# AIRLegend/ChessRL

Measured on AMD Instinct MI355X. Metric: MCTS simulations/sec at 800 sims/move, higher is better.
Workload: dtype f16

## Files before the change

### chessrl_amd/csrc/tower_x16.hpp

```cpp
#pragma once
#include "tower_common.hpp"

namespace crl_tower {

template <int F, int NB_, int SPLIT_ = 0>
struct Geo16 {
    static_assert(F == 64 || F == 128 || F == 256, "supported filter counts");
    static constexpr int SPLIT = SPLIT_;
    static constexpr int LO_OFF = F * 2;
    static constexpr int NB = NB_;
    static constexpr int WPB = 8 / NB;
    static constexpr int NT = (F == 64 && NB == 2) ? 1 : 2;
    static constexpr int CT = 2 * NT;
    static constexpr int CG = F / (16 * CT);
    static constexpr int PH = WPB / CG;
    static constexpr int PT = 4 / PH;
    static_assert(NB * CG * PH == 8 && (PH == 1 || PH == 2), "8 waves per workgroup");
    static constexpr int KT = F == 256 ? 32 : 64;
    static constexpr int SPT = KT / 32;
    static constexpr int WROW = KT * 2;
    static constexpr int WCH = WROW / 16;
    static constexpr int TILE_BYTES = F * WROW;
    static constexpr int GL = TILE_BYTES / 8192;
    static constexpr int AROW_CH = (SPLIT ? 2 * F : F) < 128 ? 128 : (SPLIT ? 2 * F : F);
    static constexpr int AROW = AROW_CH * 2 + 32;
    static constexpr int ABOARD = 64 * AROW;
    static constexpr int ZERO_OFF = NB * ABOARD;
    static constexpr int ZSTRIDE = AROW;
    static constexpr int ZERO_BYTES = 16 * ZSTRIDE;
    static constexpr int BIAS_OFF = ZERO_OFF + ZERO_BYTES;
    static constexpr int WRING_OFF = ((BIAS_OFF + 2 * F * 4 + 1023) / 1024) * 1024;
    static constexpr int LDS_BYTES = WRING_OFF + PIPE_RING * TILE_BYTES;
    static_assert(LDS_BYTES <= 160 * 1024, "LDS budget");
    static constexpr int lds_bytes(int ring) { return WRING_OFF + ring * TILE_BYTES; }
    static constexpr int WPLANE = F * 64;
    __device__ static int wswz(int row) { return (0 - (row >> 2)) & 3; }
    __host__ __device__ static constexpr int chan_of(int ct, int i)
    {
        return 32 * (ct >> 1) + 8 * (i >> 2) + 4 * (ct & 1) + (i & 3);
    }
    __host__ __device__ static constexpr int row_channel(int row)
    {
        return (row & ~31) + chan_of((row >> 4) & 1, row & 15);
    }
};

constexpr int GROUP_TAPS = 3;
template <int NB, int PAIR, int GROUP>
constexpr int ring_slots()
{
    return GROUP ? GROUP_TAPS * (NB == 2 ? 4 : 3) : (PAIR ? 5 : PIPE_RING);
}

template <class G>
__device__ inline void stage_wtile_x16(const unsigned char *wts, lds_byte *lds, int t, int tid, int wave_u,
                                       int slot = -1)
{
    const unsigned char *src = wts + (size_t)t * G::TILE_BYTES;
    const int slot0 = G::WRING_OFF + (slot < 0 ? (t & (PIPE_RING - 1)) : slot) * G::TILE_BYTES;
    const int dst0 = slot0 + wave_u * 1024;
#pragma unroll
    for (int j = 0; j < G::GL; j++) {
        const int idx = j * 512 + tid;
        const unsigned off = (unsigned)(idx * 16);
        __builtin_amdgcn_global_load_lds(
            (const __attribute__((address_space(1))) void *)(src + off),
            (__attribute__((address_space(3))) void *)(lds + dst0 + j * 8192), 16, 0, 0);
    }
}

template <class G, int F>
__device__ inline void stage_bias_x16(const float *bias, lds_byte *lds, int conv, int lane, int wave_u)
{
    if (wave_u >= F / 64) return;
    const unsigned long long a = reinterpret_cast<unsigned long long>(bias + (size_t)conv * F + wave_u * 64);
    const unsigned lo = __builtin_amdgcn_readfirstlane((unsigned)a), hi = __builtin_amdgcn_readfirstlane((unsigned)(a >> 32));
    const unsigned char *src = reinterpret_cast<const unsigned char *>(((unsigned long long)hi << 32) | lo);
    __builtin_amdgcn_global_load_lds(
        (const __attribute__((address_space(1))) void *)(src + (unsigned)(lane * 4)),
        (__attribute__((address_space(3))) void *)(lds + G::BIAS_OFF + (conv & 1) * F * 4 + wave_u * 256), 4, 0, 0);
}

typedef float f32x4v __attribute__((ext_vector_type(4)));

#ifndef CRL_TRUNK_RANKPAIR
#define CRL_TRUNK_RANKPAIR 1
#endif
template <int F, int NB, int PAIR, int GROUP, int SPLIT, int IDX>
struct RankTiles {
    static constexpr bool value = CRL_TRUNK_RANKPAIR != 0 && F == 128 && NB == 4 && PAIR == 1 && GROUP == 0 &&
                                  SPLIT == 0 && IDX == 0;
};

template <int F, int NB, int BITS = 0, int ALT = 0, int PAIR = 0, int GROUP = 0, int SPLIT = 0, int IDX = 0>
__global__ __launch_bounds__(512, 2) void k_trunk_x16(const unsigned char *__restrict__ planes,
                                                       const unsigned char *__restrict__ wts,
                                                       const float *__restrict__ bias,
                                                       float *__restrict__ out, int n_blocks,
                                                       const float *__restrict__ head_w,
                                                       const float *__restrict__ head_b,
                                                       float *__restrict__ head_out)
{
    static_assert(ALT == 0, "reserved");
    typedef Geo16<F, NB, SPLIT> G;
    static_assert(!SPLIT || !GROUP, "split precision runs the plain / pair pipelines");
    constexpr int PT = G::PT, CT = G::CT;
    extern __shared__ __attribute__((aligned(1024))) unsigned char lds_raw[];
    lds_byte *lds = (lds_byte *)lds_raw;
    const int lds_base = (int)(size_t)lds;
    const int tid = threadIdx.x, lane = tid & 63, wave = tid >> 6;
    const int board_w = wave / G::WPB;
    const int obase = (16 * CT) * ((wave / G::PH) % G::CG);
    const int pbase = 32 * (wave % G::PH);
    const int r = lane & 15, q = lane >> 4;
    const int wave_u = __builtin_amdgcn_readfirstlane(wave);
    constexpr bool RP = RankTiles<F, NB, PAIR, GROUP, SPLIT, IDX>::value;
    const int rp_half = wave_u >> 2;
    const int board = RP ? 2 * ((wave >> 1) & 1) + (r >> 3) : board_w;
    const int pos0 = RP ? (rp_half ? 56 : 0) + (r & 7) : pbase + r;
    const int pstep = RP ? (rp_half ? -8 : 8) : 16;
    const int n_convs = 1 + 2 * n_blocks;
    const int tiles_stem = 9 * (SPLIT ? 2 : 1) * (128 / G::KT), tiles_conv = 9 * (SPLIT ? 2 : 1) * (F / G::KT);
    const int n_tiles = tiles_stem + 2 * n_blocks * tiles_conv;
    const size_t wg_board0 = (size_t)blockIdx.x * G::NB;
    int rows[G::NB];
    if constexpr (IDX) {
        static_assert(BITS == 1, "the indexed launch reads plane bitboards");
        const int *list = reinterpret_cast<const int *>(out);
        const int listed = __builtin_amdgcn_readfirstlane(list[0]);
        if ((int)wg_board0 >= listed) return;
#pragma unroll
        for (int b = 0; b < G::NB; b++) {
            const int k = (int)wg_board0 + b < listed ? (int)wg_board0 + b : listed - 1;
            rows[b] = __builtin_amdgcn_readfirstlane(list[LIST_HEADER + k]);
        }
    }

    static_assert(!PAIR || F == 128 || F == 256, "pair publishing: even tile counts per layer");
    constexpr int GK = GROUP_TAPS;
    constexpr int GR = ring_slots<NB, PAIR, GROUP>();
    constexpr int GRG = GR / GK;
    static_assert(G::lds_bytes(GR) <= 160 * 1024, "LDS budget");
    static_assert(!GROUP || (F == 64 && !PAIR && G::SPT == 2 && G::GL == 1 && 2 * (PT + CT) < 16),
                  "group pipeline: 64 filters");
    stage_bias_x16<G, F>(bias, lds, 0, lane, wave_u);
    if constexpr (GROUP) {
#pragma unroll
        for (int k = 0; k < GK * (GRG - 1); k++) stage_wtile_x16<G>(wts, lds, k, tid, wave_u, k);
    } else {
        stage_wtile_x16<G>(wts, lds, 0, tid, wave_u, PAIR ? 0 : -1);
        stage_wtile_x16<G>(wts, lds, 1, tid, wave_u, PAIR ? 1 : -1);
        stage_wtile_x16<G>(wts, lds, 2, tid, wave_u, PAIR ? 2 : -1);
        if constexpr (PAIR) stage_wtile_x16<G>(wts, lds, 3, tid, wave_u, 3);
    }

    {
        if constexpr (IDX) {
            expand_bitplanes_rows<G::NB, G::AROW, G::ABOARD>(planes, lds, rows, tid);
        } else if constexpr (BITS) {
            expand_bitplanes<G::NB, G::AROW, G::ABOARD>(planes, lds, wg_board0, tid);
        } else {
            const u32x4 *src = reinterpret_cast<const u32x4 *>(planes + wg_board0 * BOARD_BYTES);
#pragma unroll
            for (int i = 0; i < G::NB * 2; i++) {
                const int c16 = i * 512 + tid;
                const int p = (c16 >> 4) & 63, c = c16 & 15, b = c16 >> 10;
                u32x4 v = src[c16];
                *reinterpret_cast<__attribute__((address_space(3))) u32x4 *>(
                    lds + b * G::ABOARD + p * G::AROW + (c << 4)) = v;
            }
        }
        for (int i = tid; i < G::ZERO_BYTES / 16; i += 512)
            *reinterpret_cast<__attribute__((address_space(3))) u32x4 *>(lds + G::ZERO_OFF + i * 16) =
                u32x4{0u, 0u, 0u, 0u};
    }
    if constexpr (GROUP) wait_vmcnt<GK * (GRG - 2)>();
    else wait_vmcnt<2 * G::GL>();
    wait_lgkm<0>();
    __builtin_amdgcn_s_barrier();
    __builtin_amdgcn_sched_barrier(0);

    const int px = r & 7, py0 = (pbase >> 3) + (r >> 3);
    const int base0 = lds_base + board * G::ABOARD + pos0 * G::AROW + q * 16;
    const int zero_q = lds_base + G::ZERO_OFF + q * 16;
    const int act_row0 = board * G::ABOARD + pos0 * G::AROW;
    const int row_step = pstep * G::AROW;
    const unsigned long long xm_left = __ballot(px >= 1), xm_right = __ballot(px <= 6);
    unsigned long long ym_up[PT], ym_down[PT];
#pragma unroll
    for (int pt = 0; pt < PT; pt++) {
        ym_up[pt] = RP ? ~0ull : __ballot(py0 + 2 * pt >= 1);
        ym_down[pt] = RP ? ~0ull : __ballot(py0 + 2 * pt <= 6);
    }
    const int w0 = lds_base + G::WRING_OFF + (obase + r) * 64 + ((q ^ G::wswz(obase + r)) << 4);
    static_assert((16 * 64) == 1024 && G::TILE_BYTES * 2 + G::WPLANE + 3 * 1024 < 65536, "ds_read immediate");

    f32x4v res[PT][CT];
#pragma unroll
    for (int a = 0; a < PT; a++)
#pragma unroll
        for (int b = 0; b < CT; b++) res[a][b] = f32x4v{-0.f, -0.f, -0.f, -0.f};

    constexpr int HP = PT / 2;

    int t = 0;
    int slot_tap = 0;
    auto slot_add = [](int s, int k) { const int x = s + k; return x >= 5 ? x - 5 : x; };
    for (int conv = 0; conv < n_convs; conv++) {
        f32x4v acc[PT][CT];
#pragma unroll
        for (int ct = 0; ct < CT; ct++) {
            const f32x4 bv = *reinterpret_cast<const __attribute__((address_space(3))) f32x4 *>(
                lds + G::BIAS_OFF + (conv & 1) * F * 4 + (obase + G::chan_of(ct, 0) + 8 * q) * 4);
#pragma unroll
            for (int pt = 0; pt < PT; pt++) acc[pt][ct] = f32x4v{bv[0], bv[1], bv[2], bv[3]};
        }
        bool bias_staged = false;

        half8 xa[HP], xb[HP], w[2][CT];
        int ab[2][PT];

        auto run_tap = [&](auto NSC, auto DUPC, bool first_tap, bool last_tap, auto SKC, auto NSKC) {
            constexpr int NS = decltype(NSC)::value, DUP = decltype(DUPC)::value;
            constexpr int SK = decltype(SKC)::value ? 1 : 0, NSK = decltype(NSKC)::value ? 1 : 0;
            static_assert(RP || (SK == 0 && NSK == 0), "whole blocks leave the board only with rank tiles");
            static_assert(DUP == 1 || (SPLIT && DUP == 2), "shared weight sub-steps belong to the split kernels");
            const int t_tap0 = t;
            auto fetch_xa = [&](auto IC, bool next_tap, auto SC) {
                constexpr int i = decltype(IC)::value;
#pragma unroll
                for (int pt = decltype(SC)::value; pt < HP; pt++)
                    xa[pt] = lds_read16_asm<(i / DUP) * 64 + (i % DUP) * G::LO_OFF>(ab[next_tap ? 1 : 0][pt]);
            };
            auto fetch_xb = [&](auto IC) {
                constexpr int i = decltype(IC)::value;
#pragma unroll
                for (int pt = 0; pt < HP; pt++)
                    xb[pt] = lds_read16_asm<(i / DUP) * 64 + (i % DUP) * G::LO_OFF>(ab[0][HP + pt]);
            };
            constexpr int NSW = NS / DUP;
            constexpr int TPT = NSW / G::SPT;
            static_assert((TPT == 1 || TPT == 2 || TPT == 4) && PIPE_RING == 4 && NSW % 2 == 0, "ring");
            int wv[PAIR ? TPT : 1], wv_nxt;
            if constexpr (PAIR) {
#pragma unroll
                for (int k = 0; k < TPT; k++) wv[k] = w0 + slot_add(slot_tap, k) * G::TILE_BYTES;
                wv_nxt = w0 + slot_add(slot_tap, TPT) * G::TILE_BYTES;
            } else {
                wv[0] = w0 + (t_tap0 & (PIPE_RING - 1)) * G::TILE_BYTES;
                wv_nxt = w0 + ((t_tap0 + TPT) & (PIPE_RING - 1)) * G::TILE_BYTES;
            }
            auto fetch_w1 = [&](auto IC, auto CC, bool next_tap, half8 (&dst)[CT]) {
                constexpr int i = decltype(IC)::value, ct = decltype(CC)::value;
                constexpr int off = ct * 1024 + (i % G::SPT) * G::WPLANE + (PAIR ? 0 : (i / G::SPT) * G::TILE_BYTES);
                dst[ct] = lds_read16_asm<off>(next_tap ? wv_nxt : wv[PAIR ? i / G::SPT : 0]);
            };
            auto fetch_w = [&](auto IC, bool next_tap, half8 (&dst)[CT]) {
                static_for<0, CT>([&](auto CC) { fetch_w1(IC, CC, next_tap, dst); });
            };
            if (first_tap) {
                fetch_xa(std::integral_constant<int, 0>{}, false, std::integral_constant<int, SK>{});
                fetch_w(std::integral_constant<int, 0>{}, false, w[0]);
            }
            static_for<0, NS>([&](auto IC) {
                constexpr int i = decltype(IC)::value;
                constexpr int wi = i / DUP;
                constexpr bool w_first = i % DUP == 0, w_last = i % DUP == DUP - 1;
                constexpr int s = wi % G::SPT;
                constexpr int cur = wi % 2, nxt = 1 - cur;
                if constexpr (!w_first) {
                } else if constexpr (PAIR) {
                    if constexpr (s == G::SPT - 1 && ((wi / G::SPT) & 1) == 1) {
                        wait_vmcnt<0>();
                        __builtin_amdgcn_s_barrier();
                        __builtin_amdgcn_sched_barrier(0);
                        if (!bias_staged) {
                            bias_staged = true;
                            if (conv + 1 < n_convs) stage_bias_x16<G, F>(bias, lds, conv + 1, lane, wave_u);
                        }
                        const int slot_cur = slot_add(slot_tap, wi / G::SPT);
                        if (t + 3 < n_tiles) stage_wtile_x16<G>(wts, lds, t + 3, tid, wave_u, slot_add(slot_cur, 3));
                        if (t + 4 < n_tiles) stage_wtile_x16<G>(wts, lds, t + 4, tid, wave_u, slot_add(slot_cur, 4));
                    }
                } else if constexpr (s == G::SPT - 1) {
                    if (t + 2 < n_tiles) wait_vmcnt<G::GL>();
                    else wait_vmcnt<0>();
                    __builtin_amdgcn_s_barrier();
                    __builtin_amdgcn_sched_barrier(0);
                    if (!bias_staged) {
                        bias_staged = true;
                        if (conv + 1 < n_convs) stage_bias_x16<G, F>(bias, lds, conv + 1, lane, wave_u);
                    }
                    if (t + 3 < n_tiles) stage_wtile_x16<G>(wts, lds, t + 3, tid, wave_u);
                }
                fetch_xb(IC);
                wait_lgkm<HP>();
                __builtin_amdgcn_sched_barrier(0);
#pragma unroll
                for (int pt = SK; pt < HP; pt++)
#pragma unroll
                    for (int ct = 0; ct < CT; ct++)
                        acc[pt][ct] = __builtin_amdgcn_mfma_f32_16x16x32_f16(w[cur][ct], xa[pt], acc[pt][ct], 0, 0, 0);
                __builtin_amdgcn_sched_barrier(0);
                constexpr bool wrap = i + 1 >= NS;
                bool issued = false;
                if (!wrap || !last_tap) {
                    issued = true;
                    if constexpr (wrap) fetch_xa(std::integral_constant<int, 0>{}, true, std::integral_constant<int, NSK>{});
                    else fetch_xa(std::integral_constant<int, i + 1>{}, false, std::integral_constant<int, SK>{});
                }
                if (!issued) wait_lgkm<0>();
                else wait_lgkm<HP - (wrap ? NSK : SK)>();
                __builtin_amdgcn_sched_barrier(0);
                static_for<0, HP * CT>([&](auto KC) {
                    constexpr int k = decltype(KC)::value, pt = k / CT, ct = k % CT;
                    acc[HP + pt][ct] = __builtin_amdgcn_mfma_f32_16x16x32_f16(w[cur][ct], xb[pt], acc[HP + pt][ct], 0, 0, 0);
                    if constexpr (k < CT && w_last) {
                        __builtin_amdgcn_sched_barrier(0);
                        if (issued) {
                            if constexpr (wrap) fetch_w1(std::integral_constant<int, 0>{}, KC, true, w[nxt]);
                            else fetch_w1(std::integral_constant<int, wi + 1>{}, KC, false, w[nxt]);
                        }
                        __builtin_amdgcn_sched_barrier(0);
                    }
                });
                __builtin_amdgcn_sched_barrier(0);
                if constexpr (s == G::SPT - 1 && w_last) t++;
            });
        };

        const int hshift = GROUP ? (conv == 0 ? 1 : 0) : ((conv != 0 && F == 256) ? 1 : 0);
        constexpr int chstep = GROUP ? 128 : 256;
        const int parts = SPLIT ? 2 : 1;
        const int per_tap = parts << hshift;
        const int nv = 9 * per_tap;
        int base0_tap = base0, r_tap = r;
        auto vtap_rows = [&](int v, int (&dst)[PT]) {
            int tap, choff;
            if constexpr (SPLIT) {
                tap = v / per_tap;
                const int rem = v - tap * per_tap;
                choff = (rem & ((1 << hshift) - 1)) * chstep;
            } else {
                tap = v >> hshift;
                choff = (v & ((1 << hshift) - 1)) * chstep;
            }
            const int dy = tap / 3 - 1, dx = tap % 3 - 1;
            const int shift = 8 * dy + dx;
            const int zrow = zero_q + ((r_tap + shift) & 15) * G::ZSTRIDE + choff;
            const int inb = base0_tap + shift * G::AROW + choff;
            const unsigned long long xm = dx < 0 ? xm_left : (dx > 0 ? xm_right : ~0ull);
#pragma unroll
            for (int pt = 0; pt < PT; pt++) {
                const unsigned long long m = xm & (dy < 0 ? ym_up[pt] : (dy > 0 ? ym_down[pt] : ~0ull));
                const int row = inb + pt * row_step;
                asm("v_cndmask_b32 %0, %1, %2, %3" : "=v"(dst[pt]) : "v"(zrow), "v"(row), "s"(m));
            }
        };
        if constexpr (GROUP) {
            constexpr int FR = PT + CT;
            half8 fx[3][PT], fw[3][CT];
            const int n_groups = n_tiles / GK;
            for (int g0 = 0; g0 < nv; g0 += GK) {
                const bool more = g0 + GK < nv;
                int rows[GK + 1][PT], wb[GK + 1];
#pragma unroll
                for (int k = 0; k <= GK; k++) {
                    vtap_rows(g0 + k < nv ? g0 + k : 0, rows[k]);
                    int slot = slot_tap + k;
                    slot = slot >= GR ? slot - GR : slot;
                    wb[k] = w0 + slot * G::TILE_BYTES;
                }
                auto fetch = [&](auto JC) {
                    constexpr int j = decltype(JC)::value, b = j % 3, k = j / 2, pl = j % 2;
#pragma unroll
                    for (int pt = 0; pt < PT; pt++) fx[b][pt] = lds_read16_asm<pl * 64>(rows[k][pt]);
                    static_for<0, CT>([&](auto CC) {
                        constexpr int ct = decltype(CC)::value;
                        fw[b][ct] = lds_read16_asm<ct * 1024 + pl * G::WPLANE>(wb[k]);
                    });
                };
                if (g0 == 0) {
                    fetch(std::integral_constant<int, 0>{});
                    fetch(std::integral_constant<int, 1>{});
                }
                static_for<0, 2 * GK>([&](auto IC) {
                    constexpr int i = decltype(IC)::value;
                    if constexpr (i == 2 * GK - 2) {
                        const int tg = t / GK;
                        if (tg + 1 < n_groups) {
                            if (tg + GRG - 2 < n_groups) wait_vmcnt<GK * (GRG - 3)>();
                            else wait_vmcnt<0>();
                            __builtin_amdgcn_s_barrier();
                            __builtin_amdgcn_sched_barrier(0);
                            if (!bias_staged) {
                                bias_staged = true;
                                if (conv + 1 < n_convs) stage_bias_x16<G, F>(bias, lds, conv + 1, lane, wave_u);
                            }
                            if (tg + GRG - 1 < n_groups) {
                                int slot = slot_tap - GK;
                                slot = slot < 0 ? slot + GR : slot;
#pragma unroll
                                for (int k = 0; k < GK; k++)
                                    stage_wtile_x16<G>(wts, lds, (tg + GRG - 1) * GK + k, tid, wave_u, slot + k);
                            }
                        }
                    }
                    if constexpr (i + 2 < 2 * GK) fetch(std::integral_constant<int, i + 2>{});
                    else if (more) fetch(std::integral_constant<int, i + 2>{});
                    if constexpr (i + 2 < 2 * GK) wait_lgkm<2 * FR>();
                    else if constexpr (i == 2 * GK - 2) { if (more) wait_lgkm<2 * FR>(); else wait_lgkm<FR>(); }
                    else { if (more) wait_lgkm<2 * FR>(); else wait_lgkm<0>(); }
                    __builtin_amdgcn_sched_barrier(0);
#pragma unroll
                    for (int pt = 0; pt < PT; pt++)
#pragma unroll
                        for (int ct = 0; ct < CT; ct++)
                            acc[pt][ct] = __builtin_amdgcn_mfma_f32_16x16x32_f16(fw[i % 3][ct], fx[i % 3][pt], acc[pt][ct], 0, 0, 0);
                    __builtin_amdgcn_sched_barrier(0);
                });
                t += GK;
                slot_tap += GK;
                slot_tap = slot_tap >= GR ? slot_tap - GR : slot_tap;
            }
        } else if constexpr (RP) {
            constexpr std::integral_constant<int, 1> once{};
            auto run_conv = [&](auto HC) {
                constexpr int hh = decltype(HC)::value;
                auto fresh = [&] {
                    base0_tap = base0;
                    r_tap = r;
                    asm volatile("" : "+v"(base0_tap), "+v"(r_tap));
                };
                fresh();
                vtap_rows(0, ab[1]);
                static_for<0, 9>([&](auto VC) {
                    constexpr int v = decltype(VC)::value;
                    constexpr bool sk = hh == 0 ? v < 3 : v >= 6;
                    constexpr bool nsk = v + 1 < 9 && (hh == 0 ? v + 1 < 3 : v + 1 >= 6);
#pragma unroll
                    for (int pt = 0; pt < PT; pt++) ab[0][pt] = ab[1][pt];
                    fresh();
                    vtap_rows(v + 1 < 9 ? v + 1 : 0, ab[1]);
                    run_tap(std::integral_constant<int, 4>{}, once, v == 0, v == 8, std::integral_constant<bool, sk>{},
                            std::integral_constant<bool, nsk>{});
                    slot_tap = slot_add(slot_tap, 4 / G::SPT);
                });
            };
            if (rp_half == 0) run_conv(std::integral_constant<int, 0>{});
            else run_conv(std::integral_constant<int, 1>{});
        } else {
        constexpr std::false_type nsk{};
        vtap_rows(0, ab[1]);
        for (int v = 0; v < nv; v++) {
#pragma unroll
            for (int pt = 0; pt < PT; pt++) ab[0][pt] = ab[1][pt];
            vtap_rows(v + 1 < nv ? v + 1 : 0, ab[1]);
            constexpr std::integral_constant<int, 1> once{};
            bool whi_twice = false;
            if constexpr (SPLIT) {
                const bool whi = ((v % per_tap) >> hshift) == 0;
                whi_twice = conv != 0 && whi;
            }
            if (whi_twice) {
                if constexpr (SPLIT) {
                    constexpr std::integral_constant<int, 2> twice{};
                    if (F == 64) run_tap(std::integral_constant<int, 4>{}, twice, v == 0, v == nv - 1, nsk, nsk);
                    else run_tap(std::integral_constant<int, 8>{}, twice, v == 0, v == nv - 1, nsk, nsk);
                }
            } else if (F == 64 && conv != 0) run_tap(std::integral_constant<int, 2>{}, once, v == 0, v == nv - 1, nsk, nsk);
            else run_tap(std::integral_constant<int, 4>{}, once, v == 0, v == nv - 1, nsk, nsk);
            if constexpr (PAIR) slot_tap = slot_add(slot_tap, 4 / G::SPT);
            if constexpr (SPLIT) wait_lgkm<0>();
        }
        }

        wait_lgkm<0>();
        __builtin_amdgcn_s_barrier();
        __builtin_amdgcn_sched_barrier(0);
        const bool conv1 = (conv & 1) != 0;
        const float floor = conv == 0 ? -__builtin_inff() : 0.f;
        auto store_pair = [&](int pt, int g, const half4 &lo, const half4 &hi) {
            *reinterpret_cast<__attribute__((address_space(3))) half8 *>(
                lds + act_row0 + pt * row_step + (obase + 32 * g + 8 * q) * 2) =
                half8{lo[0], lo[1], lo[2], lo[3], hi[0], hi[1], hi[2], hi[3]};
        };
        const half4 zero4 = {(_Float16)0, (_Float16)0, (_Float16)0, (_Float16)0};
        auto store_split = [&](int pt, int g, const f32x4v &a, const f32x4v &b) {
            half8 hi8, lo8;
#pragma unroll
            for (int j = 0; j < 4; j++) {
                hi8[j] = (_Float16)a[j];
                hi8[4 + j] = (_Float16)b[j];
                lo8[j] = (_Float16)(a[j] - (float)hi8[j]);
                lo8[4 + j] = (_Float16)(b[j] - (float)hi8[4 + j]);
            }
            lds_byte *dst = lds + act_row0 + pt * row_step + (obase + 32 * g + 8 * q) * 2;
            *reinterpret_cast<__attribute__((address_space(3))) half8 *>(dst) = hi8;
            *reinterpret_cast<__attribute__((address_space(3))) half8 *>(dst + G::LO_OFF) = lo8;
        };
        if constexpr (SPLIT) {
            auto write_layer = [&](auto value) {
#pragma unroll
                for (int g = 0; g < CT / 2; g++)
#pragma unroll
                    for (int pt = 0; pt < PT; pt++) store_split(pt, g, value(pt, 2 * g), value(pt, 2 * g + 1));
            };
            if (conv1) {
                write_layer([&](int pt, int ct) {
                    f32x4v o;
#pragma unroll
                    for (int j = 0; j < 4; j++) o[j] = fmaxf(acc[pt][ct][j], 0.f);
                    return o;
                });
                asm volatile("; conv1 written");
            } else {
                write_layer([&](int pt, int ct) {
                    const f32x4v sum = acc[pt][ct] + res[pt][ct];
#pragma unroll
                    for (int j = 0; j < 4; j++) res[pt][ct][j] = fmaxf(sum[j], floor);
                    return res[pt][ct];
                });
                asm volatile("; conv2 written");
            }
        } else
        if (conv1) {
#pragma unroll
            for (int g = 0; g < CT / 2; g++)
#pragma unroll
                for (int pt = 0; pt < PT; pt++) {
                    half4 o16[2];
#pragma unroll
                    for (int h = 0; h < 2; h++) {
#pragma unroll
                        for (int j = 0; j < 4; j++) o16[h][j] = (_Float16)acc[pt][2 * g + h][j];
                        o16[h] = __builtin_elementwise_max(o16[h], zero4);
                    }
                    store_pair(pt, g, o16[0], o16[1]);
                }
        } else {
#pragma unroll
            for (int g = 0; g < CT / 2; g++)
#pragma unroll
                for (int pt = 0; pt < PT; pt++) {
                    half4 o16[2];
#pragma unroll
                    for (int h = 0; h < 2; h++) {
                        const int ct = 2 * g + h;
                        const f32x4v sum = acc[pt][ct] + res[pt][ct];
#pragma unroll
                        for (int j = 0; j < 4; j++) {
                            const float v = fmaxf(sum[j], floor);
                            res[pt][ct][j] = v;
                            o16[h][j] = (_Float16)v;
                        }
                    }
                    store_pair(pt, g, o16[0], o16[1]);
                }
        }
        wait_lgkm<0>();
        __builtin_amdgcn_s_barrier();
        __builtin_amdgcn_sched_barrier(0);
    }
    if (!IDX && out) {
#pragma unroll
        for (int pt = 0; pt < PT; pt++) {
            const int p = pos0 + pstep * pt;
#pragma unroll
            for (int ct = 0; ct < CT; ct++) {
                const int o0 = obase + G::chan_of(ct, 0) + 8 * q;
                f32x4 v;
#pragma unroll
                for (int j = 0; j < 4; j++) v[j] = res[pt][ct][j];
                *reinterpret_cast<f32x4 *>(out + ((wg_board0 + board) * 64 + p) * F + o0) = v;
            }
        }
    }

    if (head_out) {
        constexpr int NC = 4 * G::CG;
        float part[PT][3];
#pragma unroll
        for (int pt = 0; pt < PT; pt++)
#pragma unroll
            for (int k = 0; k < 3; k++) part[pt][k] = 0.f;
#pragma unroll
        for (int ct = 0; ct < CT; ct++) {
            const int o0 = obase + G::chan_of(ct, 0) + 8 * q;
#pragma unroll
            for (int k = 0; k < 3; k++) {
                const f32x4 wv = *reinterpret_cast<const f32x4 *>(head_w + k * F + o0);
#pragma unroll
                for (int pt = 0; pt < PT; pt++)
#pragma unroll
                    for (int j = 0; j < 4; j++) part[pt][k] += res[pt][ct][j] * wv[j];
            }
        }
        __attribute__((address_space(3))) float *scratch = (__attribute__((address_space(3))) float *)lds;
#pragma unroll
        for (int pt = 0; pt < PT; pt++)
#pragma unroll
            for (int k = 0; k < 3; k++)
                scratch[(((board * 64 + pos0 + pstep * pt) * 3) + k) * NC + (obase / (16 * CT)) * 4 + q] = part[pt][k];
        wait_lgkm<0>();
        __builtin_amdgcn_s_barrier();
        for (int i = tid; i < G::NB * 64 * 3; i += 512) {
            const int k = i % 3, bp = i / 3;
            float v = 0.f;
#pragma unroll
            for (int c = 0; c < NC; c++) v += scratch[i * NC + c];
            v += head_b[k];
            size_t gb = wg_board0 + (bp >> 6);
            if constexpr (IDX) {
                gb = (size_t)rows[0];
#pragma unroll
                for (int b = 1; b < G::NB; b++) gb = (bp >> 6) == b ? (size_t)rows[b] : gb;
            }
            const int pos = bp & 63;
            head_out[gb * 192 + (k < 2 ? pos * 2 + k : 128 + pos)] = fmaxf(v, 0.f);
        }
    }
}

}
```

Baseline: 1.960 million.

## Defer and split weight-tile DMA issue into MFMA sub-steps for rank-pair half

For the rank-pair trunk kernel's second half, the global-to-LDS weight and bias staging that used to follow each tap barrier is recorded and issued later as per-piece loads. The default phase issues it at the start of the next tap's first sub-step, or after the last tap's final MFMA group. Other phases interleave the pieces between MFMAs. The intent is to keep the barrier-to-compute path short and overlap load issue with matrix work. An optional timestamp instrumentation build is also added, which adds complexity and moves ring-slot timing closer to its hazard window.

```diff
diff --git a/chessrl_amd/csrc/tower_x16.hpp b/chessrl_amd/csrc/tower_x16.hpp
--- a/chessrl_amd/csrc/tower_x16.hpp
+++ b/chessrl_amd/csrc/tower_x16.hpp
@@ -69,6 +69,18 @@
     }
 }
 
+template <class G>
+__device__ inline void stage_wpiece_x16(const unsigned char *wts, lds_byte *lds, int t, int tid, int wave_u, int slot,
+                                        int j)
+{
+    const unsigned char *src = wts + (size_t)t * G::TILE_BYTES;
+    const int dst0 = G::WRING_OFF + slot * G::TILE_BYTES + wave_u * 1024;
+    const unsigned off = (unsigned)((j * 512 + tid) * 16);
+    __builtin_amdgcn_global_load_lds(
+        (const __attribute__((address_space(1))) void *)(src + off),
+        (__attribute__((address_space(3))) void *)(lds + dst0 + j * 8192), 16, 0, 0);
+}
+
 template <class G, int F>
 __device__ inline void stage_bias_x16(const float *bias, lds_byte *lds, int conv, int lane, int wave_u)
 {
@@ -91,6 +103,44 @@
     static constexpr bool value = CRL_TRUNK_RANKPAIR != 0 && F == 128 && NB == 4 && PAIR == 1 && GROUP == 0 &&
                                   SPLIT == 0 && IDX == 0;
 };
+
+#ifndef CRL_TRUNK_DMA_PHASE
+#define CRL_TRUNK_DMA_PHASE 2
+#endif
+static_assert(CRL_TRUNK_DMA_PHASE >= -1 && CRL_TRUNK_DMA_PHASE <= 3, "CRL_TRUNK_DMA_PHASE: 0 .. 3");
+
+struct TrunkDmaSync { int t = 0, slot = 0; bool bias = false; };
+template <int HH, class P>
+struct RankHalfDma {
+    static constexpr int value = HH;
+    TrunkDmaSync &sync;
+    P &pieces;
+};
+template <class H, class A, class B>
+__device__ __forceinline__ void half_pieces(const H &, A, B) {}
+template <int HH, class P, class A, class B>
+__device__ __forceinline__ void half_pieces(const RankHalfDma<HH, P> &h, A a, B b) { h.pieces(a, b); }
+template <class H>
+__device__ __forceinline__ void half_record(const H &, bool, int, int) {}
+template <int HH, class P>
+__device__ __forceinline__ void half_record(const RankHalfDma<HH, P> &h, bool bias, int t, int slot)
+{
+    h.sync.bias = bias;
+    h.sync.t = t;
+    h.sync.slot = slot;
+}
+
+#if defined(CRL_TRUNK_STAMPS)
+__device__ unsigned long long *crl_trunk_stamp_buf = nullptr;
+__device__ __forceinline__ unsigned long long trunk_stamp()
+{
+    unsigned long long t;
+    __builtin_amdgcn_sched_barrier(0);
+    asm volatile("s_memtime %0\n\ts_waitcnt lgkmcnt(0)" : "=s"(t) :: "memory");
+    __builtin_amdgcn_sched_barrier(0);
+    return t;
+}
+#endif
 
 template <int F, int NB, int BITS = 0, int ALT = 0, int PAIR = 0, int GROUP = 0, int SPLIT = 0, int IDX = 0>
 __global__ __launch_bounds__(512, 2) void k_trunk_x16(const unsigned char *__restrict__ planes,
@@ -203,6 +253,11 @@
 
     constexpr int HP = PT / 2;
 
+#if defined(CRL_TRUNK_STAMPS)
+    static_assert(CRL_TRUNK_DMA_PHASE >= 0 && CRL_TRUNK_DMA_PHASE <= 2, "stamps: not between the MFMAs of phase 3");
+    unsigned long long st_wait = 0, st_req = 0, st_syncs = 0;
+    const unsigned long long st_t0 = trunk_stamp(), st_self = trunk_stamp() - st_t0;
+#endif
     int t = 0;
     int slot_tap = 0;
     auto slot_add = [](int s, int k) { const int x = s + k; return x >= 5 ? x - 5 : x; };
@@ -220,8 +275,15 @@
         half8 xa[HP], xb[HP], w[2][CT];
         int ab[2][PT];
 
-        auto run_tap = [&](auto NSC, auto DUPC, bool first_tap, bool last_tap, auto SKC, auto NSKC) {
+        auto run_tap = [&](auto NSC, auto DUPC, bool first_tap, bool last_tap, auto SKC, auto NSKC, auto HHC) {
             constexpr int NS = decltype(NSC)::value, DUP = decltype(DUPC)::value;
+            constexpr int DPH = (RP && decltype(HHC)::value == 1) ? CRL_TRUNK_DMA_PHASE : 0;
+            constexpr int NP = 2 * G::GL;
+            constexpr std::integral_constant<int, 0> p0{};
+            constexpr std::integral_constant<int, 1> p1{};
+            constexpr std::integral_constant<int, 2> p2{};
+            constexpr std::integral_constant<int, NP> pn{};
+            static_assert(DPH == 0 || (PAIR && NS == 4 && DUP == 1 && G::SPT == 2 && NP == 4), "one sync per tap, in sub-step 3");
             constexpr int SK = decltype(SKC)::value ? 1 : 0, NSK = decltype(NSKC)::value ? 1 : 0;
             static_assert(RP || (SK == 0 && NSK == 0), "whole blocks leave the board only with rank tiles");
             static_assert(DUP == 1 || (SPLIT && DUP == 2), "shared weight sub-steps belong to the split kernels");
@@ -271,9 +333,23 @@
                 if constexpr (!w_first) {
                 } else if constexpr (PAIR) {
                     if constexpr (s == G::SPT - 1 && ((wi / G::SPT) & 1) == 1) {
+                        if constexpr (DPH != 0) {
+                            half_record(HHC, !bias_staged, t, slot_add(slot_tap, wi / G::SPT));
+                            bias_staged = true;
+                            if constexpr (DPH < 0) half_pieces(HHC, p0, pn);
+                        }
+#if defined(CRL_TRUNK_STAMPS)
+                        const unsigned long long s0 = trunk_stamp();
+#endif
                         wait_vmcnt<0>();
                         __builtin_amdgcn_s_barrier();
                         __builtin_amdgcn_sched_barrier(0);
+#if defined(CRL_TRUNK_STAMPS)
+                        const unsigned long long s1 = trunk_stamp();
+                        st_wait += s1 - s0;
+                        st_syncs++;
+#endif
+                        if constexpr (DPH == 0) {
                         if (!bias_staged) {
                             bias_staged = true;
                             if (conv + 1 < n_convs) stage_bias_x16<G, F>(bias, lds, conv + 1, lane, wave_u);
@@ -281,6 +357,10 @@
                         const int slot_cur = slot_add(slot_tap, wi / G::SPT);
                         if (t + 3 < n_tiles) stage_wtile_x16<G>(wts, lds, t + 3, tid, wave_u, slot_add(slot_cur, 3));
                         if (t + 4 < n_tiles) stage_wtile_x16<G>(wts, lds, t + 4, tid, wave_u, slot_add(slot_cur, 4));
+#if defined(CRL_TRUNK_STAMPS)
+                        st_req += trunk_stamp() - s1;
+#endif
+                        }
                     }
                 } else if constexpr (s == G::SPT - 1) {
                     if (t + 2 < n_tiles) wait_vmcnt<G::GL>();
@@ -293,15 +373,28 @@
                     }
                     if (t + 3 < n_tiles) stage_wtile_x16<G>(wts, lds, t + 3, tid, wave_u);
                 }
+                if constexpr (DPH == 2 && i == 0) { if (!first_tap) half_pieces(HHC, p0, pn); }
                 fetch_xb(IC);
                 wait_lgkm<HP>();
                 __builtin_amdgcn_sched_barrier(0);
+                if constexpr (DPH == 3 && (i == 0 || i == NS - 1)) {
+                    const bool now = i == 0 ? !first_tap : last_tap;
+                    static_for<SK * CT, HP * CT>([&](auto KC) {
+                        constexpr int k = decltype(KC)::value, pt = k / CT, ct = k % CT;
+                        acc[pt][ct] = __builtin_amdgcn_mfma_f32_16x16x32_f16(w[cur][ct], xa[pt], acc[pt][ct], 0, 0, 0);
+                        if constexpr (k == SK * CT) { if (now) half_pieces(HHC, p0, p1); }
+                        if constexpr (k == SK * CT + 1) { if (now) half_pieces(HHC, p1, p2); }
+                    });
+                } else {
 #pragma unroll
                 for (int pt = SK; pt < HP; pt++)
 #pragma unroll
                     for (int ct = 0; ct < CT; ct++)
                         acc[pt][ct] = __builtin_amdgcn_mfma_f32_16x16x32_f16(w[cur][ct], xa[pt], acc[pt][ct], 0, 0, 0);
+                }
                 __builtin_amdgcn_sched_barrier(0);
+                if constexpr (DPH == 1 && i == NS - 1) half_pieces(HHC, p0, pn);
+                if constexpr (DPH == 2 && i == NS - 1) { if (last_tap) half_pieces(HHC, p0, pn); }
                 constexpr bool wrap = i + 1 >= NS;
                 bool issued = false;
                 if (!wrap || !last_tap) {
@@ -322,6 +415,10 @@
                             else fetch_w1(std::integral_constant<int, wi + 1>{}, KC, false, w[nxt]);
                         }
                         __builtin_amdgcn_sched_barrier(0);
+                    }
+                    if constexpr (DPH == 3 && k < 2 && (i == 0 || i == NS - 1)) {
+                        if (i == 0 ? !first_tap : last_tap)
+                            half_pieces(HHC, std::integral_constant<int, 2 + k>{}, std::integral_constant<int, 3 + k>{});
                     }
                 });
                 __builtin_amdgcn_sched_barrier(0);
@@ -434,6 +531,26 @@
                 };
                 fresh();
                 vtap_rows(0, ab[1]);
+                TrunkDmaSync dma_sync;
+                auto dma_pieces = [&](auto P0C, auto P1C) {
+                    __builtin_amdgcn_sched_barrier(0);
+#if defined(CRL_TRUNK_STAMPS)
+                    const unsigned long long s0 = trunk_stamp();
+#endif
+                    static_for<decltype(P0C)::value, decltype(P1C)::value>([&](auto PC) {
+                        constexpr int p = decltype(PC)::value, k = 3 + p / G::GL;
+                        if constexpr (p == 0) {
+                            if (dma_sync.bias && conv + 1 < n_convs) stage_bias_x16<G, F>(bias, lds, conv + 1, lane, wave_u);
+                        }
+                        if (dma_sync.t + k < n_tiles)
+                            stage_wpiece_x16<G>(wts, lds, dma_sync.t + k, tid, wave_u, slot_add(dma_sync.slot, k), p % G::GL);
+                    });
+#if defined(CRL_TRUNK_STAMPS)
+                    st_req += trunk_stamp() - s0;
+#endif
+                    __builtin_amdgcn_sched_barrier(0);
+                };
+                const RankHalfDma<hh, decltype(dma_pieces)> half{dma_sync, dma_pieces};
                 static_for<0, 9>([&](auto VC) {
                     constexpr int v = decltype(VC)::value;
                     constexpr bool sk = hh == 0 ? v < 3 : v >= 6;
@@ -443,7 +560,7 @@
                     fresh();
                     vtap_rows(v + 1 < 9 ? v + 1 : 0, ab[1]);
                     run_tap(std::integral_constant<int, 4>{}, once, v == 0, v == 8, std::integral_constant<bool, sk>{},
-                            std::integral_constant<bool, nsk>{});
+                            std::integral_constant<bool, nsk>{}, half);
                     slot_tap = slot_add(slot_tap, 4 / G::SPT);
                 });
             };
@@ -451,6 +568,7 @@
             else run_conv(std::integral_constant<int, 1>{});
         } else {
         constexpr std::false_type nsk{};
+        constexpr std::integral_constant<int, 0> nh{};
         vtap_rows(0, ab[1]);
         for (int v = 0; v < nv; v++) {
 #pragma unroll
@@ -465,11 +583,11 @@
             if (whi_twice) {
                 if constexpr (SPLIT) {
                     constexpr std::integral_constant<int, 2> twice{};
-                    if (F == 64) run_tap(std::integral_constant<int, 4>{}, twice, v == 0, v == nv - 1, nsk, nsk);
-                    else run_tap(std::integral_constant<int, 8>{}, twice, v == 0, v == nv - 1, nsk, nsk);
+                    if (F == 64) run_tap(std::integral_constant<int, 4>{}, twice, v == 0, v == nv - 1, nsk, nsk, nh);
+                    else run_tap(std::integral_constant<int, 8>{}, twice, v == 0, v == nv - 1, nsk, nsk, nh);
                 }
-            } else if (F == 64 && conv != 0) run_tap(std::integral_constant<int, 2>{}, once, v == 0, v == nv - 1, nsk, nsk);
-            else run_tap(std::integral_constant<int, 4>{}, once, v == 0, v == nv - 1, nsk, nsk);
+            } else if (F == 64 && conv != 0) run_tap(std::integral_constant<int, 2>{}, once, v == 0, v == nv - 1, nsk, nsk, nh);
+            else run_tap(std::integral_constant<int, 4>{}, once, v == 0, v == nv - 1, nsk, nsk, nh);
             if constexpr (PAIR) slot_tap = slot_add(slot_tap, 4 / G::SPT);
             if constexpr (SPLIT) wait_lgkm<0>();
         }
@@ -562,6 +680,16 @@
         __builtin_amdgcn_s_barrier();
         __builtin_amdgcn_sched_barrier(0);
     }
+#if defined(CRL_TRUNK_STAMPS)
+    if constexpr (RP) {
+        const unsigned long long st_loop = trunk_stamp() - st_t0;
+        unsigned long long *dbg = crl_trunk_stamp_buf;
+        if (lane == 0 && dbg) {
+            dbg += ((size_t)blockIdx.x * 8 + wave_u) * 5;
+            dbg[0] = st_loop; dbg[1] = st_wait; dbg[2] = st_req; dbg[3] = st_syncs; dbg[4] = st_self;
+        }
+    }
+#endif
     if (!IDX && out) {
 #pragma unroll
         for (int pt = 0; pt < PT; pt++) {
```

New measurement: 2.010 million, median of 6. 1.03x the previous value.
